# ultravideo/kvazaar

Hardware: AMD Instinct MI355X
Metric: CTUs/s (all-intra ultrafast hot path) (higher is better)
Workload: dtype u8/i16 (f64 RD costs); 1 GPU; 1920x1080 yuv420p 8-bit all-intra ultrafast CTU pass (kvz_hip_intra_frames), QP 22; ctus_per_frame=510, distinct_frames=8, wpp=True, parallelism=frames sharded over 1 GPU(s), no data-path collective

## Files before the change

### include/kvz_hip_dev.h

```cpp
#ifndef KVZ_HIP_DEV_H_
#define KVZ_HIP_DEV_H_

#include "kvz_hip_types.h"

#ifdef __cplusplus
extern "C" {
#endif

void *kvz_hip_dev_alloc(size_t bytes);
void  kvz_hip_dev_free(void *p);
void  kvz_hip_dev_upload(void *dev_dst, const void *host_src, size_t bytes);
void  kvz_hip_dev_download(void *host_dst, const void *dev_src, size_t bytes);
void  kvz_hip_dev_sync(void);
void  kvz_hip_dev_copy(void *dev_dst, const void *dev_src, size_t bytes);
void  kvz_hip_dev_timer_start(void);
float kvz_hip_dev_timer_stop(void);

int  kvz_hip_dev_sad_nxn(int n, const uint8_t *a, const uint8_t *b, int count, uint32_t *out);
int  kvz_hip_dev_satd_nxn(int n, const uint8_t *a, const uint8_t *b, int count, uint32_t *out);

int  kvz_hip_dev_transform(int kind, const int16_t *in, int16_t *tmp, int16_t *out, int count, int use_matrix_cores);

int  kvz_hip_dev_angular_pred(int log2_width, int mode, const uint8_t *ref_above, const uint8_t *ref_left, int count, uint8_t *out);

int  kvz_hip_dev_intra_select(int log2w, int nblk, const uint32_t *raw, const int8_t *preds, const double *mode_bits, int count, int32_t *winner);

int  kvz_hip_dev_cu8_units(int count, int from_coeffs, const int16_t *in, const int32_t *qp, int16_t *levels, int16_t *dequant, int16_t *resid);

void kvz_hip_dev_deblock_frames(uint8_t *frames, int width, int height, int n_frames, const uint8_t *cu_depth, int qp, int beta_offset_div2,
                                int tc_offset_div2);

typedef struct kvz_hip_cu_dbk {
  uint8_t type;
  uint8_t depth, tr_depth, part_size;
  uint8_t cbf_y;
  uint8_t mv_dir;
  int8_t  mv_ref[2];
  int16_t ref_id[2];
  int16_t mv[2][2];
} kvz_hip_cu_dbk;
void kvz_hip_dev_deblock_frames_inter(uint8_t *frames, int width, int height, int n_frames, const kvz_hip_cu_dbk *info, int qp, int beta_offset_div2,
                                      int tc_offset_div2, int slice_is_b);

int  kvz_hip_dev_loop_filters_inter(const uint8_t *src, uint8_t *rec, int width, int height, int n_pictures, const kvz_hip_cu_dbk *info, int qp, int slice_is_b, int deblock,
                                    int beta_offset_div2, int tc_offset_div2, int sao, int no_wpp, kvz_hip_sao_params *luma, kvz_hip_sao_params *chroma, uint8_t *merge);

int  kvz_hip_dev_sad_surface(const uint8_t *cur, const uint8_t *ref, int width, int height, int bw, int range, const int16_t *blk_xy, int count,
                             uint32_t *out);

typedef struct kvz_hip_fme_pu {
  int16_t x, y, w, h;
  int16_t mv_x, mv_y;
  int8_t  hpel_x, hpel_y;
  int16_t reserved;
} kvz_hip_fme_pu;
#define KVZ_HIP_FME_COSTS 17
int  kvz_hip_dev_fme_costs(const uint8_t *cur, const uint8_t *ref, int width, int height, const kvz_hip_fme_pu *pus, int count, int max_pu_size, int steps, uint32_t *out);

typedef struct kvz_hip_mc_pu {
  int16_t x, y, w, h;
// ... 113 lines not shown
```

### kvazaar_amd/csrc/kvz_ctu.hpp

```cpp
#pragma once
#include <type_traits>
#include "../../include/kvz_hip_types.h"
#include "kvz_ops.hpp"
#include "kvz_rdoq.hpp"
#include "kvz_recon.hpp"
#include "kvz_residual.hpp"
#include "kvz_select.hpp"

namespace kvz {

#define KVZ_CTU_THREADS 128
#ifdef KVZ_HOSTSIM
#define KVZ_FOR_THREADS(tid) for (int tid = 0; tid < KVZ_CTU_THREADS; ++tid)
#ifdef KVZ_HOSTSIM_COUNT_SYNCS
static unsigned long long g_kvz_syncs;
#define KVZ_SYNC() (++g_kvz_syncs)
#else
#define KVZ_SYNC()
#endif
#define KVZ_LDS_ADD(p, v) (*(p) += (v))
#else
#define KVZ_FOR_THREADS(tid) for (int tid = (threadIdx.x + lane_rot) & (KVZ_CTU_THREADS - 1), once_ = 1; once_; once_ = 0)
#define KVZ_SYNC() __syncthreads()
#define KVZ_LDS_ADD(p, v) atomicAdd((p), (v))
// ... 923 lines not shown
  KVZ_DEV static U16x2 splat16(int v) { U16x2 r; r.x = (unsigned short)v; r.y = (unsigned short)v; return r; }
  KVZ_DEV static U16x2 widen(unsigned hi, unsigned lo, unsigned sel) { return u16x2_of(__builtin_amdgcn_perm(hi, lo, sel)); }
  KVZ_DEV static Pk16 as_pk16(U16x2 v) { Pk16 r; __builtin_memcpy(&r, &v, 4); return r; }
  KVZ_DEV static void widen8(const u8 *p, U16x2 out[4])
  {
    unsigned w[2];
    __builtin_memcpy(w, p, 8);
    out[0] = widen(0, w[0], 0x0c010c00u); out[1] = widen(0, w[0], 0x0c030c02u); out[2] = widen(0, w[1], 0x0c010c00u); out[3] = widen(0, w[1], 0x0c030c02u);
  }
#endif
  template <bool PAIR>
  KVZ_DEV u32 angular_block_satd(int log2w, int mode, int bx, int by, int xl, int yl, int half) const
  {
    const int w = 1 << log2w;
    const bool big = S32 && log2w == 5;
    const bool flat = mode < 2;
    const bool vertical = mode >= 18 || flat;
    const int disp = s->mode_disp[mode];
    const int p0 = vertical ? bx : by, q0 = vertical ? by : bx;
    const u8 *mr;
    if (disp < 0) mr = big ? mref32() + (mode - 11) * KVZ_MREF32_STRIDE + KVZ_MREF32_ORG : s->mref[mode - 11] + KVZ_MREF_ORG;
    else {
      const bool filt = imin(iabs(mode - 26), iabs(mode - 10)) > (log2w == 3 ? 7 : (log2w == 4 ? 1 : 0));
      mr = filt ? s->fref[vertical ? 0 : 1] : s->ref[0][vertical ? 0 : 1];
    }
    mr += p0 + 1;
    const u8 *org = vertical ? org_at(0, xl + bx, yl + by) : (big ? org_t32() : s->org_t) + bx * w + by;
    const int ostride = vertical ? 32 : w;
    const u8 *side = vertical ? s->ref[0][1] : s->ref[0][0];
    const bool edge = !big && !flat && disp == 0 && p0 == 0;
    constexpr int NR = PAIR ? 4 : 8;
    const int r0 = PAIR ? 4 * half : 0;
    Pk16 d[NR][4];
#ifndef KVZ_HOSTSIM
    if (!big) {
      if (flat) {
        if (mode == 0) {
          const u8 *top = s->fref[0], *left = s->fref[1];
          const int tr = top[w + 1], bl = left[w + 1];
          U16x2 tp[4], xs[4];
          widen8(top + bx + 1, tp);
#pragma unroll
          for (int j = 0; j < 4; j++) { xs[j].x = (unsigned short)(bx + 2 * j); xs[j].y = (unsigned short)(bx + 2 * j + 1); }
#pragma unroll
          for (int i = 0; i < NR; i++) {
            const int y = by + r0 + i, l = left[y + 1];
            const U16x2 dl = splat16(tr - l), wy = splat16(w - 1 - y), hb = splat16((w - 1) * l + tr + (y + 1) * bl + w);
            U16x2 o[4];
            widen8(org + (r0 + i) * ostride, o);
#pragma unroll
            for (int j = 0; j < 4; j++) d[i][j] = as_pk16(((xs[j] * dl + (tp[j] * wy + hb)) >> (unsigned short)(log2w + 1)) - o[j]);
          }
        } else {
          const u8 *top = s->ref[0][0], *left = s->ref[0][1];
          const int dc = s->dcval[0];
          U16x2 tp[4];
          widen8(top + bx + 1, tp);
#pragma unroll
          for (int i = 0; i < NR; i++) {
            const int y = by + r0 + i;
            U16x2 o[4], v[4];
            widen8(org + (r0 + i) * ostride, o);
#pragma unroll
            for (int j = 0; j < 4; j++) v[j] = y == 0 ? (U16x2)((tp[j] + splat16(3 * dc + 2)) >> (unsigned short)2) : splat16(dc);
            if (bx == 0) v[0].x = (unsigned short)(y == 0 ? (left[1] + 2 * dc + top[1] + 2) >> 2 : (left[y + 1] + 3 * dc + 2) >> 2);
#pragma unroll
            for (int j = 0; j < 4; j++) d[i][j] = as_pk16(v[j] - o[j]);
          }
        }
      } else {
        unsigned rnd_bits = 0x00100010u;
        asm("" : "+v"(rnd_bits));
#pragma unroll
        for (int i = 0; i < NR; i++) {
          const int qa = q0 + r0 + i + 1, delta = qa * disp, di = delta >> 5, df = delta & 31;
          const u8 *m = mr + di;
          unsigned mw[2];
          __builtin_memcpy(mw, m, 8);
          const unsigned m8 = m[8];
          const U16x2 c1 = splat16(df), c0 = splat16(32 - df), rnd = u16x2_of(rnd_bits);
          U16x2 pa[4], pb[4], o[4];
          pa[0] = widen(0, mw[0], 0x0c010c00u); pa[1] = widen(0, mw[0], 0x0c030c02u); pa[2] = widen(0, mw[1], 0x0c010c00u); pa[3] = widen(0, mw[1], 0x0c030c02u);
          pb[0] = widen(0, mw[0], 0x0c020c01u); pb[1] = widen(mw[1], mw[0], 0x0c040c03u); pb[2] = widen(0, mw[1], 0x0c020c01u); pb[3] = widen(m8, mw[1], 0x0c040c03u);
          widen8(org + (r0 + i) * ostride, o);
          U16x2 v[4];
#pragma unroll
          for (int j = 0; j < 4; j++) v[j] = (pa[j] * c0 + (pb[j] * c1 + rnd)) >> (unsigned short)5;
          if (edge) v[0].x = (unsigned short)iclip(0, 255, (int)v[0].x + (((int)side[qa] - (int)side[0]) >> 1));
#pragma unroll
          for (int j = 0; j < 4; j++) d[i][j] = as_pk16(v[j] - o[j]);
        }
      }
    } else
#endif
    {
#pragma unroll
    for (int i = 0; i < NR; i++) {
      const int r = r0 + i;
      const int qa = q0 + r + 1, delta = qa * disp, di = delta >> 5, df = delta & 31;
      const u8 *m = mr + di;
      unsigned long long ow;
      __builtin_memcpy(&ow, __builtin_assume_aligned(org + r * ostride, 8), 8);
      int v[8];
      if (flat) {
        const int y = by + r;
        if (mode == 1) {
          const u8 *top = s->ref[0][0], *left = s->ref[0][1];
          const int dc = s->dcval[0];
          for (int k = 0; k < 8; k++) v[k] = big ? dc : (int)filtered_dc_pixel(dc, bx + k, y, top, left);
        } else {
          const u8 *top = s->fref[0], *left = s->fref[1];
          for (int k = 0; k < 8; k++) v[k] = planar_pixel(log2w, bx + k, y, top, left);
        }
      } else {
        int a = m[0];
        for (int k = 0; k < 8; k++) {
          const int b = m[k + 1];
          v[k] = ((32 - df) * a + df * b + 16) >> 5;
          a = b;
        }
      }
      if (edge) v[0] = iclip(0, 255, v[0] + (((int)side[qa] - (int)side[0]) >> 1));
      for (int j = 0; j < 4; j++) d[i][j] = pk_make(v[2 * j] - (int)((ow >> (16 * j)) & 0xff), v[2 * j + 1] - (int)((ow >> (16 * j + 8)) & 0xff));
    }
    }
#ifndef KVZ_HOSTSIM
    if (PAIR ? half == 0 : true) d[0][0] = pk_add(d[0][0], KVZ_PK_BIAS);
#endif
#pragma unroll
    for (int i = 0; i < NR; i++) {
      const Pk16 a0 = pk_add(d[i][0], d[i][2]), a1 = pk_add(d[i][1], d[i][3]), a2 = pk_sub(d[i][0], d[i][2]), a3 = pk_sub(d[i][1], d[i][3]);
      d[i][0] = pk_add(a0, a1); d[i][1] = pk_sub(a0, a1); d[i][2] = pk_add(a2, a3); d[i][3] = pk_sub(a2, a3);
    }
    u32 sum = 0;
    if constexpr (PAIR) {
#ifndef KVZ_HOSTSIM
      const Pk16 sgn = pk_make(half ? -1 : 1, half ? -1 : 1);
#pragma unroll
      for (int j = 0; j < 4; j++) {
        Pk16 e[4];
#pragma unroll
        for (int i = 0; i < 4; i++) {
          int mine;
          __builtin_memcpy(&mine, &d[i][j], 4);
          const int theirs = __builtin_amdgcn_update_dpp(0, mine, 0xB1 , 0xF, 0xF, true);
          Pk16 o;
          __builtin_memcpy(&o, &theirs, 4);
          e[i] = o * sgn + d[i][j];
        }
        const Pk16 b0 = pk_add(e[0], e[2]), b1 = pk_add(e[1], e[3]), b2 = pk_sub(e[0], e[2]), b3 = pk_sub(e[1], e[3]);
        sum = pk_abs2_biased(pk_add(b0, b1), sum); sum = pk_abs2_biased(pk_sub(b0, b1), sum); sum = pk_abs2_biased(pk_add(b2, b3), sum); sum = pk_abs2_biased(pk_sub(b2, b3), sum);
      }
      sum += (u32)__builtin_amdgcn_update_dpp(0, (int)sum, 0xB1, 0xF, 0xF, true);
      return sum;
#endif
    } else {
      for (int j = 0; j < 4; j++) {
        const Pk16 a0 = pk_add(d[0][j], d[4 % NR][j]), a1 = pk_add(d[1][j], d[5 % NR][j]), a2 = pk_add(d[2][j], d[6 % NR][j]), a3 = pk_add(d[3][j], d[7 % NR][j]);
        const Pk16 a4 = pk_sub(d[0][j], d[4 % NR][j]), a5 = pk_sub(d[1][j], d[5 % NR][j]), a6 = pk_sub(d[2][j], d[6 % NR][j]), a7 = pk_sub(d[3][j], d[7 % NR][j]);
        const Pk16 b0 = pk_add(a0, a2), b1 = pk_add(a1, a3), b2 = pk_sub(a0, a2), b3 = pk_sub(a1, a3);
        const Pk16 b4 = pk_add(a4, a6), b5 = pk_add(a5, a7), b6 = pk_sub(a4, a6), b7 = pk_sub(a5, a7);
#ifdef KVZ_HOSTSIM
        sum += pk_absmax(pk_add(b0, b1)) + pk_absmax(pk_sub(b0, b1)) + pk_absmax(pk_add(b2, b3)) + pk_absmax(pk_sub(b2, b3));
        sum += pk_absmax(pk_add(b4, b5)) + pk_absmax(pk_sub(b4, b5)) + pk_absmax(pk_add(b6, b7)) + pk_absmax(pk_sub(b6, b7));
#else
        sum = pk_abs2_biased(pk_add(b0, b1), sum); sum = pk_abs2_biased(pk_sub(b0, b1), sum); sum = pk_abs2_biased(pk_add(b2, b3), sum); sum = pk_abs2_biased(pk_sub(b2, b3), sum);
        sum = pk_abs2_biased(pk_add(b4, b5), sum); sum = pk_abs2_biased(pk_sub(b4, b5), sum); sum = pk_abs2_biased(pk_add(b6, b7), sum); sum = pk_abs2_biased(pk_sub(b6, b7), sum);
#endif
      }
#ifndef KVZ_HOSTSIM
      return sum;
#endif
    }
    return 2 * sum;
  }

#ifndef KVZ_HOSTSIM
  KVZ_DEV u32 flat_block_satd8(int log2w, int mode, int bx, int by, int xl, int yl, int lane) const
  {
    const int w = 1 << log2w, r = lane & 7, y = by + r;
    U16x2 o[4], v[4];
    widen8(org_at(0, xl + bx, yl + y), o);
    if (mode == 0) {
      const u8 *top = s->fref[0], *left = s->fref[1];
      const int tr = top[w + 1], bl = left[w + 1], l = left[y + 1];
      U16x2 tp[4];
      widen8(top + bx + 1, tp);
      const U16x2 dl = splat16(tr - l), wy = splat16(w - 1 - y), hb = splat16((w - 1) * l + tr + (y + 1) * bl + w);
#pragma unroll
      for (int j = 0; j < 4; j++) {
        U16x2 xs;
        xs.x = (unsigned short)(bx + 2 * j); xs.y = (unsigned short)(bx + 2 * j + 1);
        v[j] = (xs * dl + (tp[j] * wy + hb)) >> (unsigned short)(log2w + 1);
      }
    } else if (mode == 1) {
      const u8 *top = s->ref[0][0], *left = s->ref[0][1];
      const int dc = s->dcval[0];
      U16x2 tp[4];
      widen8(top + bx + 1, tp);
#pragma unroll
      for (int j = 0; j < 4; j++) v[j] = y == 0 ? (U16x2)((tp[j] + splat16(3 * dc + 2)) >> (unsigned short)2) : splat16(dc);
      if (bx == 0) v[0].x = (unsigned short)(y == 0 ? (left[1] + 2 * dc + top[1] + 2) >> 2 : (left[y + 1] + 3 * dc + 2) >> 2);
    } else {
      widen8(s->fref[0] + bx + y + 2, v);
    }
    Pk16 d[4];
#pragma unroll
    for (int j = 0; j < 4; j++) d[j] = as_pk16(v[j] - o[j]);
    if (r == 0) d[0] = pk_add(d[0], KVZ_PK_BIAS);
    {
// ... 152 lines not shown
          const int p = t >> 1, mode = p >> 4, b = p & 15;
          const u32 v = angular_block_satd<true>(5, mode, (b & 3) * 8, (b >> 2) * 8, xl, yl, t & 1);
          if (!(t & 1)) KVZ_LDS_ADD(&s->satd_raw[mode][0], (v + 2) >> 2);
        }
#endif
      }
    } else {
    KVZ_FOR_THREADS(tid) {
#ifdef KVZ_HOSTSIM
      if (log2w == 3) build_mref<3>(tid); else build_mref<4>(tid);
#else
      if (log2w == 3) build_mref<3>(tid, mref_pre); else build_mref<4>(tid, mref_pre);
#endif
      for (int e = tid; e < w * w; e += KVZ_CTU_THREADS) {
        const int ex = e >> log2w, ey = e & (w - 1);
        s->org_t[e] = *org_at(0, xl + ex, yl + ey);
      }
      if (tid == KVZ_CTU_THREADS - 1) {
        int left, above;
        neighbour_pair(lv, x, y, &left, &above);
        mpm_candidates(y, left, above, s->preds);
      }
    }
    KVZ_SYNC();
    KVZ_PROF(KVZ_P_PRED35);
    KVZ_FOR_THREADS(tid) {
      const int lb = 2 * (log2w - 3);
#ifdef KVZ_HOSTSIM
      for (int t = tid; t < 35 * nblk; t += KVZ_CTU_THREADS) {
        const int mi = t >> lb, mode = mi < 33 ? mi + 2 : mi - 33, b = t & (nblk - 1), bx = (b & ((w >> 3) - 1)) * 8, by = (b >> (log2w - 3)) * 8;
        s->satd_raw[mode][b] = angular_block_satd<false>(log2w, mode, bx, by, xl, yl, 0);
      }
#else
      if (log2w == 4) {
        const int mode = 2 + (tid >> 2), b = tid & 3;
        s->satd_raw[mode][b] = angular_block_satd<false>(4, mode, (b & 1) * 8, (b >> 1) * 8, xl, yl, 0);
      } else
      for (int t = tid; t < 64 * nblk; t += KVZ_CTU_THREADS) {
        const int p = t >> 1, mode = 2 + (p >> lb), b = p & (nblk - 1), bx = (b & ((w >> 3) - 1)) * 8, by = (b >> (log2w - 3)) * 8;
        const u32 v = angular_block_satd<true>(log2w, mode, bx, by, xl, yl, t & 1);
        if (!(t & 1)) s->satd_raw[mode][b] = v;
      }
      {
        const int t = KVZ_CTU_THREADS - 1 - tid;
        if (t < 24 * nblk) {
          const int mb = t >> 3, mi = mb >> lb, mode = mi == 0 ? 34 : mi - 1, b = mb & (nblk - 1), bx = (b & ((w >> 3) - 1)) * 8, by = (b >> (log2w - 3)) * 8;
          const u32 v = flat_block_satd8(log2w, mode, bx, by, xl, yl, tid);
          if ((tid & 7) == 0) s->satd_raw[mode][b] = v;
        }
      }
#endif
    }
    }
    KVZ_SYNC();
    KVZ_PROF(KVZ_P_SATD);
    KVZ_FOR_THREADS(tid) {
      if (tid >= kHookThread && tid < kHookThread + kCostEntries) cu_cost_prepare(lv, x, y, depth, tid - kHookThread);
      const int final_mode = replay_selection(tid, log2w, nblk);
      if (final_mode >= 0) {
        if (tid == 0) s->best_mode = final_mode;
#ifdef KVZ_HOSTSIM
        const int holders = 1;
#else
        const int holders = 64;
#endif
        for (int i = tid; i < (w >> 3) * (w >> 3); i += holders) {
          const int cell = ((yl >> 3) + (i >> (log2w - 3))) * 8 + (xl >> 3) + (i & ((w >> 3) - 1));
          CtuCu *cu = &s->cu[lv][cell];
          cu->type = 1; cu->depth = (u8)depth; cu->mode = (u8)final_mode; cu->tr_depth = (u8)depth;
          set_mode4(lv, cell, final_mode);
        }
      }
    }
    KVZ_SYNC();
// ... 1828 lines not shown
```

### kvazaar_amd/csrc/kvz_dev.hpp

```cpp
#pragma once
#include <hip/hip_runtime.h>

#include <functional>
#include <mutex>
#include <chrono>
#include <vector>

#include "../../include/kvz_hip_dev.h"
#include "kvz_mfma.hpp"
#include "kvz_ops.hpp"
#include "kvz_sao.hpp"
#include "kvz_entropy.hpp"
#include "kvz_select.hpp"
#include "kvz_recon.hpp"
#include "kvz_tables.hpp"

namespace kvz {

__device__ __forceinline__ u32 load_u32_any(const u8 *p) { u32 v; __builtin_memcpy(&v, p, 4); return v; }
template <int G> __device__ __forceinline__ u32 group_sum(u32 v)
{
  for (int off = G / 2; off > 0; off >>= 1) v += __shfl_down(v, off, G);
  return v;
}
// ... 252 lines not shown
  else if (stage == 2) { if (!from_coeffs) t1[e] = cu8_fwd_first<L2>(t0, e, fwd); }
  else if (stage == 3) {
    int level = 0, dq = in[po + e];
    if (!from_coeffs) {
      const QuantScalars q = quant_scalars(qp, 8, 1, 0, 1 << L2, c ? 2 : 0);
      level = quant_level(cu8_fwd_second<L2>(t1, e, fwd), q);
      dq = dequant_level(level, q);
    }
    levels[po + e] = (i16)level;
    dequant[po + e] = (i16)dq;
    t0[cu8_transposed<L2>(e)] = (i16)dq;
  }
  else if (stage == 4) t1[cu8_transposed<L2>(e)] = cu8_inv_first<L2>(t0, e, inv);
  else resid[po + e] = cu8_inv_second<L2>(t1, e, inv);
}
__global__ void __launch_bounds__(256) dev_cu8_units_kernel(const i16 *in, const int32_t *qp, const int count, const int from_coeffs, const Tables *tb, i16 *levels, i16 *dequant, i16 *resid)
{
  __shared__ alignas(16) i16 t[2][2][96];
  const int half = threadIdx.x >> 7, tid = threadIdx.x & 127;
  const long unit = 2l * blockIdx.x + half, o = 96 * unit;
  const bool live = unit < count && tid < 96;
  const int c = tid < 64 ? 0 : (tid < 80 ? 1 : 2), e = tid < 64 ? tid : (tid & 15), q = live ? qp[unit] : 0;
  Cu8MatRow fwd = {}, inv = {};
  if (tid < 64) cu8_matrix_rows<3>(tb, e, fwd, inv); else cu8_matrix_rows<2>(tb, e, fwd, inv);
  for (int stage = 1; stage <= 5; stage++) {
    if (live) {
      if (tid < 64) dev_cu8_lane<3>(stage, c, e, t[half], from_coeffs, q, fwd, inv, in + o, levels + o, dequant + o, resid + o);
      else dev_cu8_lane<2>(stage, c, e, t[half], from_coeffs, q, fwd, inv, in + o, levels + o, dequant + o, resid + o);
    }
    __syncthreads();
  }
}

template <int L2> __global__ void __launch_bounds__(256) dev_angular_kernel(const u8 *above, const u8 *left, const int count, const int mode, u8 *out)
{
  constexpr int W = 1 << L2, NG = kAngularGroupsPerLane, GPB = W * W / 4, BLOCKS = 256 * NG / GPB, RS = 2 * W + 1, ES = (2 * W + 1 + 8 + 3) & ~3;
  constexpr int RAW = (BLOCKS * RS + 3 + 3) / 4 + 2;
  __shared__ u32 s_raw[2][RAW];
  __shared__ alignas(8) u8 s_ext[BLOCKS][ES];
  __shared__ u32 s_tile[BLOCKS * W * W / 4];
  const int disp_tab[9] = { 0, 2, 5, 9, 13, 17, 21, 26, 32 };
  const int inv_tab[9] = { 0, 4096, 1638, 910, 630, 482, 390, 315, 256 };
  const bool vertical = mode >= 18;
  const int mode_disp = vertical ? mode - 26 : 10 - mode, ad = iabs(mode_disp);
  const int disp = mode_disp < 0 ? -disp_tab[ad] : disp_tab[ad], inv = inv_tab[ad];
  const long blk0 = (long)blockIdx.x * BLOCKS;
  const int nblk = (int)(count - blk0 < BLOCKS ? count - blk0 : BLOCKS);
  const long g0 = blk0 * RS;
  const int mis = (int)(g0 & 3), ndw = (mis + nblk * RS + 3) >> 2;
  const u8 *main_g = vertical ? above : left, *side_g = vertical ? left : above;
  const int tid = threadIdx.x;
  for (int i = tid; i < ndw; i += 256) {
    s_raw[0][i] = reinterpret_cast<const u32 *>(main_g + g0 - mis)[i];
    if (disp < 0) s_raw[1][i] = reinterpret_cast<const u32 *>(side_g + g0 - mis)[i];
  }
  __syncthreads();
  if (disp < 0) {
    const int lowest = (W * disp) >> 5, span = W + 1 - lowest;
    const u8 *rm = reinterpret_cast<const u8 *>(s_raw[0]) + mis, *rs = reinterpret_cast<const u8 *>(s_raw[1]) + mis;
    constexpr int LPB = BLOCKS >= 256 ? 1 : 256 / BLOCKS;
    for (int bb = tid / LPB; bb < nblk; bb += 256 / LPB)
      for (int j = tid % LPB; j < span; j += LPB) {
        const int k = j + lowest;
        s_ext[bb][k + W] = k >= -1 ? rm[bb * RS + k + 1] : rs[bb * RS + ((128 + (-1 - k) * inv) >> 8)];
      }
    __syncthreads();
// ... 827 lines not shown
  if (!tmp) { fprintf(stderr, "kvz_hip_dev_transform: the scalar path needs tmp\n"); return -1; }
  A::transform_dev(be(), kind, 8, in, tmp, out, count);
  return 0;
}

int kvz_hip_dev_angular_pred(int log2_width, int mode, const uint8_t *ref_above, const uint8_t *ref_left, int count, uint8_t *out)
{
  if (count <= 0) return 0;
  const int blocks_per_wg = 256 * kvz::kAngularGroupsPerLane / ((1 << (2 * log2_width)) / 4);
  const long threads = ((long)count + blocks_per_wg - 1) / blocks_per_wg * 256;
  switch (log2_width) {
  case 2: KVZ_DEV_LAUNCH(kvz::dev_angular_kernel<2>, threads, ref_above, ref_left, count, mode, out); break;
  case 3: KVZ_DEV_LAUNCH(kvz::dev_angular_kernel<3>, threads, ref_above, ref_left, count, mode, out); break;
  case 4: KVZ_DEV_LAUNCH(kvz::dev_angular_kernel<4>, threads, ref_above, ref_left, count, mode, out); break;
  case 5: KVZ_DEV_LAUNCH(kvz::dev_angular_kernel<5>, threads, ref_above, ref_left, count, mode, out); break;
  default: fprintf(stderr, "kvz_hip_dev_angular_pred: unsupported log2_width=%d\n", log2_width); return -1;
  }
  return 0;
}

int kvz_hip_dev_intra_select(int log2w, int nblk, const uint32_t *raw, const int8_t *preds, const double *mode_bits, int count, int32_t *winner)
{
  if (!((log2w == 3 && nblk == 1) || (log2w == 4 && nblk == 4))) { fprintf(stderr, "kvz_hip_dev_intra_select: unsupported log2w=%d nblk=%d\n", log2w, nblk); return -1; }
  if (count <= 0) return 0;
  KVZ_DEV_LAUNCH(kvz::dev_intra_select_kernel, ((long)count + 3) / 4 * 256, raw, preds, mode_bits, count, log2w, nblk, winner);
  return 0;
}

int kvz_hip_dev_cu8_units(int count, int from_coeffs, const int16_t *in, const int32_t *qp, int16_t *levels, int16_t *dequant, int16_t *resid)
{
  if (count < 0 || (from_coeffs != 0 && from_coeffs != 1)) { fprintf(stderr, "kvz_hip_dev_cu8_units: count=%d from_coeffs=%d\n", count, from_coeffs); return -1; }
  if (count == 0) return 0;
  KVZ_DEV_LAUNCH(kvz::dev_cu8_units_kernel, ((long)count + 1) / 2 * 256, in, qp, count, from_coeffs, kvz::device_tables(), levels, dequant, resid);
  return 0;
}

void kvz_hip_dev_deblock_frames(uint8_t *frames, int width, int height, int n_frames, const uint8_t *cu_depth, int qp, int beta_offset_div2,
                                int tc_offset_div2)
{
  kvz::deblock_frames_on(be().stream, frames, width, height, n_frames, cu_depth, qp, beta_offset_div2, tc_offset_div2);
}

void kvz_hip_dev_deblock_frames_inter(uint8_t *frames, int width, int height, int n_frames, const kvz_hip_cu_dbk *info, int qp, int beta_offset_div2, int tc_offset_div2,
                                      int slice_is_b)
{
  kvz::deblock_frames_on(be().stream, frames, width, height, n_frames, nullptr, qp, beta_offset_div2, tc_offset_div2, 3, info, slice_is_b);
}

namespace kvz {
struct LoopScratch {
  u8 *ver = nullptr, *dbk = nullptr; size_t pic_bytes = 0;
  SaoStats *stats = nullptr; SaoCand *cand = nullptr; SaoRec *recs = nullptr; u8 *merge = nullptr; size_t lcus = 0;
  float *fbits = nullptr;
  int32_t *qps = nullptr; size_t n_qps = 0;
  SaoQpRow *sao_rows = nullptr;
};
inline LoopScratch &loop_scratch()
{
  static thread_local LoopScratch s[64];
  static thread_local bool registered = false;
  if (!registered) {
    registered = true;
    LoopScratch *all = s;
    thread_state().cleanups.push_back([all]() {
      for (int d = 0; d < 64; d++) {
        LoopScratch &x = all[d];
// ... 1010 lines not shown
```

### kvazaar_amd/csrc/kvz_mfma.hpp

```cpp
#pragma once
#include <hip/hip_runtime.h>

#include "kvz_ops.hpp"

namespace kvz {

typedef int dev_int4 __attribute__((ext_vector_type(4)));
typedef int dev_int16 __attribute__((ext_vector_type(16)));

__device__ __forceinline__ void dev_byte_planes(int v0, int v1, int v2, int v3, u32 &lo, u32 &hi)
{
  const u32 t01 = __builtin_amdgcn_perm((u32)v1, (u32)v0, 0x05010400u), t23 = __builtin_amdgcn_perm((u32)v3, (u32)v2, 0x05010400u);
  lo = __builtin_amdgcn_perm(t23, t01, 0x05040100u) ^ 0x80808080u;
  hi = __builtin_amdgcn_perm(t23, t01, 0x07060302u);
}

template <int N> struct DevMma;
template <> struct DevMma<16> {
  static constexpr int NREG = 4;
  static __device__ __forceinline__ int idx(int lane) { return lane & 15; }
  static __device__ __forceinline__ int row(int lane, int r) { return 4 * (lane >> 4) + r; }
  static __device__ __forceinline__ int k0(int lane, int) { return 4 * (lane >> 4); }
  static constexpr int STEPS = 1;
};
// ... 93 lines not shown
      for (int i = 0; i < 4; i++) v[4 * st + i] = x[(M::k0(lane, st) + i) * N + col];
    dev_product<N>(v, Tt, sTt, false, lane, 64, t);
    for (int r = 0; r < M::NREG; r++) v[r] = iclip(-32768, 32767, t[r] >> 7);
    dev_product<N>(v, Tt, sTt, false, lane, 2048, t);
    for (int r = 0; r < M::NREG; r++) o[M::row(lane, r) * N + col] = (i16)iclip(-32768, 32767, t[r] >> 12);
  }
}

template <int NB> __device__ __forceinline__ void mfma_transform_blocks16(const i16 *x, i16 *o, bool inverse, const Tables *tb, int lane)
{
  typedef DevMma<16> M;
  const int col = M::idx(lane), k0 = M::k0(lane, 0);
  const DevTable16 t = dev_table16(tb->dct_i8[0][inverse ? 1 : 0], tb->dct_sum[0][inverse ? 1 : 0], lane);
  int v[NB][4], w[NB][4];
  const u16 *xu = reinterpret_cast<const u16 *>(x);
#pragma unroll
  for (int b = 0; b < NB; b++) {
    u32 l, h;
    if (!inverse) {
      const uint2 q = *reinterpret_cast<const uint2 *>(x + b * 256 + col * 16 + k0);
      l = __builtin_amdgcn_perm(q.y, q.x, 0x06040200u) ^ 0x80808080u;
      h = __builtin_amdgcn_perm(q.y, q.x, 0x07050301u);
    } else dev_byte_planes((int)xu[b * 256 + k0 * 16 + col], (int)xu[b * 256 + (k0 + 1) * 16 + col], (int)xu[b * 256 + (k0 + 2) * 16 + col], (int)xu[b * 256 + (k0 + 3) * 16 + col], l, h);
    dev_product16_planes(l, h, t, false, inverse ? 64 : 4, w[b]);
  }
#pragma unroll
  for (int b = 0; b < NB; b++) for (int r = 0; r < 4; r++) v[b][r] = inverse ? iclip(-32768, 32767, w[b][r] >> 7) : w[b][r] >> 3;
#pragma unroll
  for (int b = 0; b < NB; b++) dev_product16(v[b], t, !inverse, inverse ? 2048 : 512, w[b]);
#pragma unroll
  for (int b = 0; b < NB; b++) for (int r = 0; r < 4; r++) o[b * 256 + M::row(lane, r) * 16 + col] = (i16)(inverse ? iclip(-32768, 32767, w[b][r] >> 12) : w[b][r] >> 10);
}

}
```

### kvazaar_amd/csrc/kvz_ops.hpp

```cpp
#pragma once
#include <stdint.h>

#ifdef KVZ_HOSTSIM
#define KVZ_DEV inline
#define KVZ_ATOMIC_ADD(p, v) (*(p) += (v))
#else
#include <hip/hip_runtime.h>
#define KVZ_DEV __device__ __forceinline__
#define KVZ_ATOMIC_ADD(p, v) atomicAdd((p), (v))
#endif

namespace kvz {

typedef uint8_t u8;
typedef int16_t i16;
typedef uint16_t u16;
typedef uint32_t u32;
typedef int32_t i32;

#ifdef KVZ_HOSTSIM
#define KVZ_HD inline
#else
#define KVZ_HD __host__ __device__ __forceinline__
#endif
// ... 13 lines not shown
  return __builtin_amdgcn_sdot2(va, vb, c, false);
}
#endif
#ifndef KVZ_HOSTSIM
KVZ_DEV int row16_sum(int v)
{
  v += __builtin_amdgcn_update_dpp(0, v, 0x118, 0xF, 0xF, true);
  v += __builtin_amdgcn_update_dpp(0, v, 0x114, 0xF, 0xF, true);
  v += __builtin_amdgcn_update_dpp(0, v, 0x112, 0xF, 0xF, true);
  v += __builtin_amdgcn_update_dpp(0, v, 0x111, 0xF, 0xF, true);
  return v;
}
#endif

constexpr unsigned kMrefStride = 36, kMrefOrg = 16, kMrefRefRow = 68, kMrefFiltered = 408;

struct Tables {
  i16 dct[4][32 * 32];
  i16 dst4[16];
  alignas(16) int8_t dct_i8[2][2][32 * 32];
  alignas(16) i32 dct_sum[2][2][32];
  alignas(16) int8_t bd_i8[3][2][16 * 16];
  alignas(16) i32 bd_sum[3][2][16];
  u32 small_pairs[3][2][8][4];
  u32 pairs16[2][16][8];
  u32 scan[3][4][1024];
  u8 avail_top[16][16], avail_left[16][16];
  u8 ctx_next[2][128];
  u32 mref_tab[2][512];
  u8 diag8[64];
  u32 entropy_bits[128];
  int8_t luma_filter[4][8];
  int8_t chroma_filter[8][4];
};


struct SadRectOp {
  const u8 *a; int a_stride; long a_bstride;
  const u8 *b; int b_stride; long b_bstride;
  int w, h;
  int clamp, ref_w, ref_h, ref_x, ref_y;
  u32 *out;
  KVZ_DEV void operator()(int item) const
  {
    const int blk = item / h, y = item - blk * h;
    const u8 *pa = a + blk * a_bstride + (long)y * a_stride;
    u32 s = 0;
    if (!clamp) {
      const u8 *pb = b + blk * b_bstride + (long)y * b_stride;
      for (int x = 0; x < w; x++) s += iabs((int)pa[x] - (int)pb[x]);
    } else {
      const int ry = iclip(0, ref_h - 1, ref_y + y);
      const u8 *pb = b + blk * b_bstride + (long)ry * b_stride;
      for (int x = 0; x < w; x++) s += iabs((int)pa[x] - (int)pb[iclip(0, ref_w - 1, ref_x + x)]);
    }
    KVZ_ATOMIC_ADD(&out[blk], s);
  }
};

struct HorSadOp {
  const u8 *pic; int pic_stride; const u8 *ref; int ref_stride; int w, h, left, right; u32 *out;
  KVZ_DEV void operator()(int y) const
  {
    const u8 *p = pic + (long)y * pic_stride, *r = ref + (long)y * ref_stride;
    u32 s = 0;
    for (int x = 0; x < w; x++) {
      int rx = x;
// ... 557 lines not shown
```

### kvazaar_amd/csrc/kvz_tables.hpp

```cpp
#pragma once
#include <string.h>

#include "kvz_recon.hpp"
#include "kvz_syntax.hpp"

namespace kvz {

inline int dct32_entry(int k, int n)
{
  static const int mag[32] = { 64, 90, 90, 90, 89, 88, 87, 85, 83, 82, 80, 78, 75, 73, 70, 67,
                               64, 61, 57, 54, 50, 46, 43, 38, 36, 31, 25, 22, 18, 13, 9,  4 };
  if (k == 0) return 64;
  const int m = (k * (2 * n + 1)) % 128;
  if (m < 32) return mag[m];
  if (m < 64) return -mag[64 - m];
  if (m < 96) return -mag[m - 64];
  return mag[128 - m];
}

inline void scan_pattern(int type, int size, int *xs, int *ys)
{
  int n = 0;
  if (type == 0) {
    for (int d = 0; d < 2 * size - 1; d++)
// ... 67 lines not shown
        else { for (int cc = c; cc < 16 && z(cc, r - 1) < z(c, r); cc++) n++; t->avail_top[r][c] = (u8)(4 * n); }
        n = 0;
        if (c == 0) t->avail_left[r][c] = (u8)(64 - 4 * r);
        else { for (int rr = r; rr < 16 && z(c - 1, rr) < z(c, r); rr++) n++; t->avail_left[r][c] = (u8)(4 * n); }
      }
  }
  {
    static const u8 lps[64] = { 0, 0, 1, 2, 2, 4, 4, 5, 6, 7, 8, 9, 9, 11, 11, 12, 13, 13, 15, 15, 16, 16, 18, 18, 19, 19, 21, 21, 22, 22, 23, 24,
                                24, 25, 26, 26, 27, 27, 28, 29, 29, 30, 30, 30, 31, 32, 32, 33, 33, 33, 34, 34, 35, 35, 35, 36, 36, 36, 37, 37, 37, 38, 38, 63 };
    for (int u = 0; u < 128; u++) {
      const int st = u >> 1, mps = u & 1;
      t->ctx_next[0][u] = (u8)(st >= 62 ? u : ((st + 1) << 1) | mps);
      t->ctx_next[1][u] = (u8)(st == 0 ? (mps ^ 1) : (lps[st] << 1) | mps);
    }
  }
  {
    int n = 0;
    for (int d = 0; d < 15; d++) for (int x = 0; x <= d; x++) if (x < 8 && d - x < 8) t->diag8[n++] = (u8)((d - x) * 8 + x);
  }
  for (int l2 = 3; l2 <= 4; l2++) {
    static const int inv_tab[9] = { 0, 4096, 1638, 910, 630, 482, 390, 315, 256 };
    const int w = 1 << l2, nq = 2 * w + 2;
    for (int i = 0; i < 15 * nq; i++) {
      const int mode = 11 + i / nq, q = i % nq - w, vertical = mode >= 18, md = vertical ? mode - 26 : 10 - mode, ad = md < 0 ? -md : md;
      const bool filt = luma_reads_filtered(l2, mode);
      int idx = q >= 0 ? q : (128 + (-q) * inv_tab[ad]) >> 8;
      if (idx > 2 * w) idx = 2 * w;
      const int main_side = vertical ? 0 : 1, side = q >= 0 ? main_side : 1 - main_side;
      const unsigned src = (filt ? kMrefFiltered : 0u) + kMrefRefRow * side + idx, dst = kMrefStride * (i / nq) + kMrefOrg + i % nq - w;
      t->mref_tab[l2 - 3][i] = src | dst << 16;
    }
    for (int i = 15 * nq; i < 512; i++) t->mref_tab[l2 - 3][i] = t->mref_tab[l2 - 3][15 * nq - 1];
  }
  static const i16 dst4[16] = { 29, 55, 74, 84, 74, 74, 0, -74, 84, -29, -74, 55, 55, -84, 74, -29 };
  memcpy(t->dst4, dst4, sizeof dst4);
  for (int kind = 0; kind < 3; kind++) {
    const int n = kind == 1 ? 8 : 4;
    const i16 *m = kind == 2 ? t->dst4 : t->dct[kind == 1 ? 1 : 0];
    for (int g = 0; g < 16 / n; g++)
      for (int k = 0; k < n; k++)
        for (int j = 0; j < n; j++) {
          t->bd_i8[kind][0][(g * n + k) * 16 + g * n + j] = (int8_t)m[k * n + j];
          t->bd_i8[kind][1][(g * n + j) * 16 + g * n + k] = (int8_t)m[k * n + j];
          t->bd_sum[kind][0][g * n + k] += m[k * n + j];
          t->bd_sum[kind][1][g * n + j] += m[k * n + j];
        }
  }
  for (int kind = 0; kind < 3; kind++) {
    const int n = kind == 1 ? 8 : 4;
    const i16 *m = kind == 2 ? t->dst4 : t->dct[kind == 1 ? 1 : 0];
    for (int k = 0; k < n; k++)
      for (int i = 0; i < n / 2; i++) {
        t->small_pairs[kind][0][k][i] = (u32)(u16)m[k * n + 2 * i] | ((u32)(u16)m[k * n + 2 * i + 1] << 16);
        t->small_pairs[kind][1][k][i] = (u32)(u16)m[(2 * i) * n + k] | ((u32)(u16)m[(2 * i + 1) * n + k] << 16);
      }
  }
  for (int k = 0; k < 16; k++)
    for (int i = 0; i < 8; i++) {
      const i16 *m = t->dct[2];
      t->pairs16[0][k][i] = (u32)(u16)m[k * 16 + 2 * i] | ((u32)(u16)m[k * 16 + 2 * i + 1] << 16);
      t->pairs16[1][k][i] = (u32)(u16)m[(2 * i) * 16 + k] | ((u32)(u16)m[(2 * i + 1) * 16 + k] << 16);
    }
  for (int type = 0; type < 3; type++)
    for (int l2 = 2; l2 <= 5; l2++) {
      const int size = 1 << l2, cgs = size / 4;
      int gx[64], gy[64], px[16], py[16], n = 0;
// ... 83 lines not shown
```

### kvazaar_amd/dev.py

```python
import ctypes as C

import numpy as np

TRANSFORM_KINDS = {"dct4": 0, "dct8": 1, "dct16": 2, "dct32": 3, "dst4": 4, "idct4": 5, "idct8": 6, "idct16": 7, "idct32": 8, "idst4": 9}
TRANSFORM_SIZE = {0: 4, 1: 8, 2: 16, 3: 32, 4: 4, 5: 4, 6: 8, 7: 16, 8: 32, 9: 4}


class Dev:
    def __init__(self, cdll):
        self.lib = l = cdll
        vp, sz, ci = C.c_void_p, C.c_size_t, C.c_int
        l.kvz_hip_dev_alloc.restype = vp; l.kvz_hip_dev_alloc.argtypes = [sz]
        l.kvz_hip_dev_free.restype = None; l.kvz_hip_dev_free.argtypes = [vp]
        l.kvz_hip_dev_upload.restype = None; l.kvz_hip_dev_upload.argtypes = [vp, vp, sz]
        l.kvz_hip_dev_download.restype = None; l.kvz_hip_dev_download.argtypes = [vp, vp, sz]
        l.kvz_hip_dev_sync.restype = None; l.kvz_hip_dev_sync.argtypes = []
        l.kvz_hip_dev_timer_start.restype = None; l.kvz_hip_dev_timer_start.argtypes = []
        l.kvz_hip_dev_timer_stop.restype = C.c_float; l.kvz_hip_dev_timer_stop.argtypes = []
        for f in (l.kvz_hip_dev_sad_nxn, l.kvz_hip_dev_satd_nxn):
            f.restype = None; f.argtypes = [ci, vp, vp, ci, vp]
        l.kvz_hip_dev_transform.restype = None; l.kvz_hip_dev_transform.argtypes = [ci, vp, vp, vp, ci, ci]
        l.kvz_hip_dev_angular_pred.restype = None; l.kvz_hip_dev_angular_pred.argtypes = [ci, ci, vp, vp, ci, vp]
        l.kvz_hip_dev_intra_select.restype = ci; l.kvz_hip_dev_intra_select.argtypes = [ci, ci, vp, vp, vp, ci, vp]
        l.kvz_hip_dev_cu8_units.restype = ci; l.kvz_hip_dev_cu8_units.argtypes = [ci, ci, vp, vp, vp, vp, vp]

    def put(self, a):
        a = np.ascontiguousarray(a)
        p = self.lib.kvz_hip_dev_alloc(a.nbytes)
        self.lib.kvz_hip_dev_upload(p, a.ctypes.data, a.nbytes)
        return p

    def copy_in(self, p, a):
        a = np.ascontiguousarray(a)
        self.lib.kvz_hip_dev_upload(p, a.ctypes.data, a.nbytes)

    def empty(self, nbytes):
        return self.lib.kvz_hip_dev_alloc(nbytes)

    def get(self, p, shape, dtype):
        out = np.empty(shape, dtype)
        self.lib.kvz_hip_dev_download(out.ctypes.data, p, out.nbytes)
        return out

    def free(self, *ps):
        for p in ps:
            self.lib.kvz_hip_dev_free(p)
```

Baseline: 3.260 million CTUs/s.

## Compute angular 8x8 SATD for intra search with int8 MFMA Walsh transforms

```diff
diff --git a/include/kvz_hip_dev.h b/include/kvz_hip_dev.h
--- a/include/kvz_hip_dev.h
+++ b/include/kvz_hip_dev.h
@@ -26,6 +26,8 @@
 int  kvz_hip_dev_intra_select(int log2w, int nblk, const uint32_t *raw, const int8_t *preds, const double *mode_bits, int count, int32_t *winner);
 
 int  kvz_hip_dev_cu8_units(int count, int from_coeffs, const int16_t *in, const int32_t *qp, int16_t *levels, int16_t *dequant, int16_t *resid);
+
+int  kvz_hip_dev_satd8_blocks(const uint8_t *a, const uint8_t *b, int count, uint32_t *out);
 
 void kvz_hip_dev_deblock_frames(uint8_t *frames, int width, int height, int n_frames, const uint8_t *cu_depth, int qp, int beta_offset_div2,
                                 int tc_offset_div2);
diff --git a/kvazaar_amd/csrc/kvz_ctu.hpp b/kvazaar_amd/csrc/kvz_ctu.hpp
--- a/kvazaar_amd/csrc/kvz_ctu.hpp
+++ b/kvazaar_amd/csrc/kvz_ctu.hpp
@@ -979,68 +979,6 @@
     constexpr int NR = PAIR ? 4 : 8;
     const int r0 = PAIR ? 4 * half : 0;
     Pk16 d[NR][4];
-#ifndef KVZ_HOSTSIM
-    if (!big) {
-      if (flat) {
-        if (mode == 0) {
-          const u8 *top = s->fref[0], *left = s->fref[1];
-          const int tr = top[w + 1], bl = left[w + 1];
-          U16x2 tp[4], xs[4];
-          widen8(top + bx + 1, tp);
-#pragma unroll
-          for (int j = 0; j < 4; j++) { xs[j].x = (unsigned short)(bx + 2 * j); xs[j].y = (unsigned short)(bx + 2 * j + 1); }
-#pragma unroll
-          for (int i = 0; i < NR; i++) {
-            const int y = by + r0 + i, l = left[y + 1];
-            const U16x2 dl = splat16(tr - l), wy = splat16(w - 1 - y), hb = splat16((w - 1) * l + tr + (y + 1) * bl + w);
-            U16x2 o[4];
-            widen8(org + (r0 + i) * ostride, o);
-#pragma unroll
-            for (int j = 0; j < 4; j++) d[i][j] = as_pk16(((xs[j] * dl + (tp[j] * wy + hb)) >> (unsigned short)(log2w + 1)) - o[j]);
-          }
-        } else {
-          const u8 *top = s->ref[0][0], *left = s->ref[0][1];
-          const int dc = s->dcval[0];
-          U16x2 tp[4];
-          widen8(top + bx + 1, tp);
-#pragma unroll
-          for (int i = 0; i < NR; i++) {
-            const int y = by + r0 + i;
-            U16x2 o[4], v[4];
-            widen8(org + (r0 + i) * ostride, o);
-#pragma unroll
-            for (int j = 0; j < 4; j++) v[j] = y == 0 ? (U16x2)((tp[j] + splat16(3 * dc + 2)) >> (unsigned short)2) : splat16(dc);
-            if (bx == 0) v[0].x = (unsigned short)(y == 0 ? (left[1] + 2 * dc + top[1] + 2) >> 2 : (left[y + 1] + 3 * dc + 2) >> 2);
-#pragma unroll
-            for (int j = 0; j < 4; j++) d[i][j] = as_pk16(v[j] - o[j]);
-          }
-        }
-      } else {
-        unsigned rnd_bits = 0x00100010u;
-        asm("" : "+v"(rnd_bits));
-#pragma unroll
-        for (int i = 0; i < NR; i++) {
-          const int qa = q0 + r0 + i + 1, delta = qa * disp, di = delta >> 5, df = delta & 31;
-          const u8 *m = mr + di;
-          unsigned mw[2];
-          __builtin_memcpy(mw, m, 8);
-          const unsigned m8 = m[8];
-          const U16x2 c1 = splat16(df), c0 = splat16(32 - df), rnd = u16x2_of(rnd_bits);
-          U16x2 pa[4], pb[4], o[4];
-          pa[0] = widen(0, mw[0], 0x0c010c00u); pa[1] = widen(0, mw[0], 0x0c030c02u); pa[2] = widen(0, mw[1], 0x0c010c00u); pa[3] = widen(0, mw[1], 0x0c030c02u);
-          pb[0] = widen(0, mw[0], 0x0c020c01u); pb[1] = widen(mw[1], mw[0], 0x0c040c03u); pb[2] = widen(0, mw[1], 0x0c020c01u); pb[3] = widen(m8, mw[1], 0x0c040c03u);
-          widen8(org + (r0 + i) * ostride, o);
-          U16x2 v[4];
-#pragma unroll
-          for (int j = 0; j < 4; j++) v[j] = (pa[j] * c0 + (pb[j] * c1 + rnd)) >> (unsigned short)5;
-          if (edge) v[0].x = (unsigned short)iclip(0, 255, (int)v[0].x + (((int)side[qa] - (int)side[0]) >> 1));
-#pragma unroll
-          for (int j = 0; j < 4; j++) d[i][j] = as_pk16(v[j] - o[j]);
-        }
-      }
-    } else
-#endif
-    {
 #pragma unroll
     for (int i = 0; i < NR; i++) {
       const int r = r0 + i;
@@ -1070,7 +1008,6 @@
       if (edge) v[0] = iclip(0, 255, v[0] + (((int)side[qa] - (int)side[0]) >> 1));
       for (int j = 0; j < 4; j++) d[i][j] = pk_make(v[2 * j] - (int)((ow >> (16 * j)) & 0xff), v[2 * j + 1] - (int)((ow >> (16 * j + 8)) & 0xff));
     }
-    }
 #ifndef KVZ_HOSTSIM
     if (PAIR ? half == 0 : true) d[0][0] = pk_add(d[0][0], KVZ_PK_BIAS);
 #endif
@@ -1123,6 +1060,52 @@
   }
 
 #ifndef KVZ_HOSTSIM
+  KVZ_DEV u32 angular_group_satd(const SatdWalsh &wm, int log2w, int mode, int bx, int by, int xl, int yl, int half) const
+  {
+    const int w = 1 << log2w;
+    const bool vertical = mode >= 18;
+    const int disp = s->mode_disp[mode];
+    const int p0 = vertical ? bx : by, q0 = vertical ? by : bx;
+    const u8 *mr;
+    if (disp < 0) mr = s->mref[mode - 11] + KVZ_MREF_ORG;
+    else {
+      const bool filt = imin(iabs(mode - 26), iabs(mode - 10)) > (log2w == 3 ? 7 : 1);
+      mr = filt ? s->fref[vertical ? 0 : 1] : s->ref[0][vertical ? 0 : 1];
+    }
+    mr += p0 + 1;
+    const u8 *org = vertical ? org_at(0, xl + bx, yl + by) : s->org_t + bx * w + by;
+    const int ostride = vertical ? 32 : w;
+    const u8 *side = vertical ? s->ref[0][1] : s->ref[0][0];
+    const bool edge = disp == 0 && p0 == 0;
+    const int r0 = 4 * half;
+    unsigned rnd_bits = 0x10101010u;
+    asm("" : "+v"(rnd_bits));
+    dev_int4 p[2], o[2];
+#pragma unroll
+    for (int i = 0; i < 4; i++) {
+      const int qa = q0 + r0 + i + 1, delta = qa * disp, di = delta >> 5, df = delta & 31;
+      const u8 *m = mr + di;
+      unsigned mw[2], ow[2];
+      __builtin_memcpy(mw, m, 8);
+      const unsigned m8 = m[8];
+      __builtin_memcpy(ow, org + (r0 + i) * ostride, 8);
+      const U16x2 c1 = splat16(df), c0 = splat16(32 - df), rnd = u16x2_of(rnd_bits);
+      const U16x2 e0 = widen(0, mw[0], 0x0c020c00u), o0 = widen(0, mw[0], 0x0c030c01u), f0 = widen(mw[1], mw[0], 0x0c040c02u);
+      const U16x2 e1 = widen(0, mw[1], 0x0c020c00u), o1 = widen(0, mw[1], 0x0c030c01u), f1 = widen(m8, mw[1], 0x0c040c02u);
+      U16x2 v[4];
+      v[0] = (e0 * c0 + (o0 * c1 + rnd)) >> (unsigned short)5; v[1] = (o0 * c0 + (f0 * c1 + rnd)) >> (unsigned short)5;
+      v[2] = (e1 * c0 + (o1 * c1 + rnd)) >> (unsigned short)5; v[3] = (o1 * c0 + (f1 * c1 + rnd)) >> (unsigned short)5;
+      if (edge) v[0].x = (unsigned short)iclip(128, 128 + 255, (int)v[0].x + (((int)side[qa] - (int)side[0]) >> 1));
+      unsigned vw[4];
+      __builtin_memcpy(vw, v, 16);
+      p[i >> 1][2 * (i & 1)] = (int)__builtin_amdgcn_perm(vw[1], vw[0], 0x06020400u);
+      p[i >> 1][2 * (i & 1) + 1] = (int)__builtin_amdgcn_perm(vw[3], vw[2], 0x06020400u);
+      o[i >> 1][2 * (i & 1)] = (int)(ow[0] ^ 0x80808080u);
+      o[i >> 1][2 * (i & 1) + 1] = (int)(ow[1] ^ 0x80808080u);
+    }
+    return satd8_group_mfma(wm, p, o);
+  }
+
   KVZ_DEV u32 flat_block_satd8(int log2w, int mode, int bx, int by, int xl, int yl, int lane) const
   {
     const int w = 1 << log2w, r = lane & 7, y = by + r;
@@ -1341,14 +1324,14 @@
         s->satd_raw[mode][b] = angular_block_satd<false>(log2w, mode, bx, by, xl, yl, 0);
       }
 #else
-      if (log2w == 4) {
-        const int mode = 2 + (tid >> 2), b = tid & 3;
-        s->satd_raw[mode][b] = angular_block_satd<false>(4, mode, (b & 1) * 8, (b >> 1) * 8, xl, yl, 0);
-      } else
-      for (int t = tid; t < 64 * nblk; t += KVZ_CTU_THREADS) {
-        const int p = t >> 1, mode = 2 + (p >> lb), b = p & (nblk - 1), bx = (b & ((w >> 3) - 1)) * 8, by = (b >> (log2w - 3)) * 8;
-        const u32 v = angular_block_satd<true>(log2w, mode, bx, by, xl, yl, t & 1);
-        if (!(t & 1)) s->satd_raw[mode][b] = v;
+      if (log2w == 4 || tid < 64) {
+        const int lane = tid & 63;
+        const SatdWalsh wm = satd8_walsh(tb, lane);
+        for (int g = log2w == 4 ? 2 * (tid >> 6) : 0, ge = g + (log2w == 4 ? 2 : 1); g < ge; g++) {
+          const int p = 32 * g + (lane & 31), mode = 2 + (p >> lb), b = p & (nblk - 1), bx = (b & ((w >> 3) - 1)) * 8, by = (b >> (log2w - 3)) * 8;
+          const u32 v = angular_group_satd(wm, log2w, mode, bx, by, xl, yl, lane >> 5);
+          if (lane < 32) s->satd_raw[mode][b] = v;
+        }
       }
       {
         const int t = KVZ_CTU_THREADS - 1 - tid;
diff --git a/kvazaar_amd/csrc/kvz_dev.hpp b/kvazaar_amd/csrc/kvz_dev.hpp
--- a/kvazaar_amd/csrc/kvz_dev.hpp
+++ b/kvazaar_amd/csrc/kvz_dev.hpp
@@ -308,6 +308,11 @@
   }
 }
 
+__global__ void __launch_bounds__(256) dev_satd8_blocks_kernel(const Tables *tb, const u8 *a, const u8 *b, const int count, u32 *out)
+{
+  dev_satd8_blocks_wave(tb, a, b, count, out, (int)(blockIdx.x * 4 + (threadIdx.x >> 6)), (int)(threadIdx.x & 63));
+}
+
 template <int L2> __global__ void __launch_bounds__(256) dev_angular_kernel(const u8 *above, const u8 *left, const int count, const int mode, u8 *out)
 {
   constexpr int W = 1 << L2, NG = kAngularGroupsPerLane, GPB = W * W / 4, BLOCKS = 256 * NG / GPB, RS = 2 * W + 1, ES = (2 * W + 1 + 8 + 3) & ~3;
@@ -1201,6 +1206,13 @@
   if (count < 0 || (from_coeffs != 0 && from_coeffs != 1)) { fprintf(stderr, "kvz_hip_dev_cu8_units: count=%d from_coeffs=%d\n", count, from_coeffs); return -1; }
   if (count == 0) return 0;
   KVZ_DEV_LAUNCH(kvz::dev_cu8_units_kernel, ((long)count + 1) / 2 * 256, in, qp, count, from_coeffs, kvz::device_tables(), levels, dequant, resid);
+  return 0;
+}
+
+int kvz_hip_dev_satd8_blocks(const uint8_t *a, const uint8_t *b, int count, uint32_t *out)
+{
+  if (count < 0) { fprintf(stderr, "kvz_hip_dev_satd8_blocks: count=%d\n", count); return -1; }
+  KVZ_DEV_LAUNCH(kvz::dev_satd8_blocks_kernel, ((long)count + 31) / 32 * 64, kvz::device_tables(), a, b, count, out);
   return 0;
 }
 
diff --git a/kvazaar_amd/csrc/kvz_mfma.hpp b/kvazaar_amd/csrc/kvz_mfma.hpp
--- a/kvazaar_amd/csrc/kvz_mfma.hpp
+++ b/kvazaar_amd/csrc/kvz_mfma.hpp
@@ -149,4 +149,48 @@
   for (int b = 0; b < NB; b++) for (int r = 0; r < 4; r++) o[b * 256 + M::row(lane, r) * 16 + col] = (i16)(inverse ? iclip(-32768, 32767, w[b][r] >> 12) : w[b][r] >> 10);
 }
 
+struct SatdWalsh { dev_int4 pos, neg; };
+constexpr int kSatdBias = 1 << 15;
+__device__ __forceinline__ SatdWalsh satd8_walsh(const Tables *tb, int lane)
+{
+  const dev_int4 *row = reinterpret_cast<const dev_int4 *>(tb->satd_walsh[lane]);
+  SatdWalsh w;
+  w.pos = row[0];
+  w.neg = row[1];
+  return w;
 }
+__device__ __forceinline__ u32 satd8_group_mfma(const SatdWalsh &w, const dev_int4 p[2], const dev_int4 o[2])
+{
+  u32 sums[2] = { 0, 0 };
+#pragma unroll
+  for (int tile = 0; tile < 2; tile++) {
+    dev_int16 t;
+#pragma unroll
+    for (int r = 0; r < 16; r++) t[r] = kSatdBias;
+    t = __builtin_amdgcn_mfma_i32_32x32x32_i8(tile ? w.neg : w.pos, p[1], t, 0, 0, 0);
+    t = __builtin_amdgcn_mfma_i32_32x32x32_i8(w.pos, p[0], t, 0, 0, 0);
+    t = __builtin_amdgcn_mfma_i32_32x32x32_i8(tile ? w.pos : w.neg, o[1], t, 0, 0, 0);
+    t = __builtin_amdgcn_mfma_i32_32x32x32_i8(w.neg, o[0], t, 0, 0, 0);
+#pragma unroll
+    for (int r = 0; r < 16; r++) sums[r & 1] = __builtin_amdgcn_sad_u16((u32)t[r], (u32)kSatdBias, sums[r & 1]);
+  }
+  const u32 sum = sums[0] + sums[1];
+  const auto both = __builtin_amdgcn_permlane32_swap(sum, sum, false, false);
+  return both[0] + both[1];
+}
+__device__ __forceinline__ void dev_satd8_blocks_wave(const Tables *tb, const u8 *a, const u8 *bsrc, int count, u32 *out, int group, int lane)
+{
+  const long blk = 32l * group + (lane & 31);
+  const bool live = blk < count;
+  dev_int4 p[2] = {}, o[2] = {};
+  if (live) {
+    const dev_int4 *pa = reinterpret_cast<const dev_int4 *>(a + 64 * blk + 32 * (lane >> 5)), *po = reinterpret_cast<const dev_int4 *>(bsrc + 64 * blk + 32 * (lane >> 5));
+    p[0] = pa[0]; p[1] = pa[1]; o[0] = po[0]; o[1] = po[1];
+  }
+#pragma unroll
+  for (int q = 0; q < 2; q++) { p[q] ^= (int)0x80808080u; o[q] ^= (int)0x80808080u; }
+  const u32 v = satd8_group_mfma(satd8_walsh(tb, lane), p, o);
+  if (live && lane < 32) out[blk] = v;
+}
+
+}
diff --git a/kvazaar_amd/csrc/kvz_ops.hpp b/kvazaar_amd/csrc/kvz_ops.hpp
--- a/kvazaar_amd/csrc/kvz_ops.hpp
+++ b/kvazaar_amd/csrc/kvz_ops.hpp
@@ -69,7 +69,16 @@
   u32 entropy_bits[128];
   int8_t luma_filter[4][8];
   int8_t chroma_filter[8][4];
-};
+  alignas(16) u32 satd_walsh[64][8];
+};
+
+KVZ_HD u32 satd_walsh_word(int lane, int q)
+{
+  const int i = lane & 31, h = lane >> 5;
+  const u32 base = 0x01010101u ^ ((i & 1) ? 0xfe00fe00u : 0u) ^ ((i & 2) ? 0xfefe0000u : 0u);
+  const int minus = (((i >> 4) & h) ^ ((i >> 3) & (q >> 1)) ^ ((i >> 2) & q)) & 1;
+  return base ^ (minus ? 0xfefefefeu : 0u);
+}
 
 
 struct SadRectOp {
diff --git a/kvazaar_amd/csrc/kvz_tables.hpp b/kvazaar_amd/csrc/kvz_tables.hpp
--- a/kvazaar_amd/csrc/kvz_tables.hpp
+++ b/kvazaar_amd/csrc/kvz_tables.hpp
@@ -123,6 +123,8 @@
     }
     for (int i = 15 * nq; i < 512; i++) t->mref_tab[l2 - 3][i] = t->mref_tab[l2 - 3][15 * nq - 1];
   }
+  for (int lane = 0; lane < 64; lane++)
+    for (int q = 0; q < 4; q++) { t->satd_walsh[lane][q] = satd_walsh_word(lane, q); t->satd_walsh[lane][4 + q] = satd_walsh_word(lane, q) ^ 0xfefefefeu; }
   static const i16 dst4[16] = { 29, 55, 74, 84, 74, 74, 0, -74, 84, -29, -74, 55, 55, -84, 74, -29 };
   memcpy(t->dst4, dst4, sizeof dst4);
   for (int kind = 0; kind < 3; kind++) {
diff --git a/kvazaar_amd/dev.py b/kvazaar_amd/dev.py
--- a/kvazaar_amd/dev.py
+++ b/kvazaar_amd/dev.py
@@ -23,6 +23,7 @@
         l.kvz_hip_dev_angular_pred.restype = None; l.kvz_hip_dev_angular_pred.argtypes = [ci, ci, vp, vp, ci, vp]
         l.kvz_hip_dev_intra_select.restype = ci; l.kvz_hip_dev_intra_select.argtypes = [ci, ci, vp, vp, vp, ci, vp]
         l.kvz_hip_dev_cu8_units.restype = ci; l.kvz_hip_dev_cu8_units.argtypes = [ci, ci, vp, vp, vp, vp, vp]
+        l.kvz_hip_dev_satd8_blocks.restype = ci; l.kvz_hip_dev_satd8_blocks.argtypes = [vp, vp, ci, vp]
 
     def put(self, a):
         a = np.ascontiguousarray(a)
```

After: 3.368 million CTUs/s, median of 6. 3.3% higher.
